# drtconway/zotmer

Hardware: AMD Instinct MI355X
Metric: Gk-mers/sec kmerize k=25 on synthetic 150bp FASTQ; achieved HBM GB/s fraction (higher is better)
Workload: dtype u64

## Files before the change

### zotmer_amd/csrc/stream_pass.hip

```cpp
#include "internal.hpp"
#include "encode_tile.hpp"

#include <stdlib.h>
#include <type_traits>

namespace zk {

constexpr int P0_BLOCK = 512, P0_NW = 8, P0_TILE = P0_BLOCK * P0_NW, P0_IMG_WORDS = 320;
constexpr int PW_BLOCK = 1024, PW_NW = 8, PW_TILE = PW_BLOCK * PW_NW, PW_IMG_WORDS = 640;
constexpr int SH_BLOCK = 512, SH_NW = 16, SH_TILE = SH_BLOCK * SH_NW;

struct P0Geom { u32 block, nw, img_words; };
__host__ __device__ constexpr P0Geom p0_geom(bool wide) { return wide ? P0Geom{PW_BLOCK, PW_NW, PW_IMG_WORDS} : P0Geom{P0_BLOCK, P0_NW, P0_IMG_WORDS}; }

struct StreamTiling {
    u32 rec;
    u32 rpt, cpr, wpr;
    u32 cpr_inv;
    u32 tile_bytes;
    u32 ranges;
    u64 range_bytes;
};

__host__ __device__ inline StreamTiling make_tiling(u64 n_bytes, u64 first_nl, int K, u32 ranges, P0Geom g) {
    StreamTiling t = {};
    const u32 tile = g.block * g.nw;
    t.ranges = ranges ? ranges : 1;
    t.tile_bytes = tile;
    if (first_nl < 0x7fffffffull) {
        const u64 rec = first_nl + 1;
        const long long W = (long long)first_nl - K + 1;
        if (rec >= 16 && W >= 1 && n_bytes % rec == 0) {
            const u32 cpr = (u32)((W + g.nw - 1) / g.nw);
            u32 rpt = cpr <= g.block ? (g.block / cpr) / 16 * 16 : 0;
            const u32 fit = (u32)((16ull * (g.img_words - 3)) / rec) / 16 * 16;
            if (rpt > fit) rpt = fit;
            if (rpt >= 16 && (u64)rpt * rec * 50 > (u64)tile * 51) {
                t.rec = (u32)rec; t.rpt = rpt; t.cpr = cpr; t.wpr = (u32)W;
                t.cpr_inv = (u32)(((1ull << 32) + cpr - 1) / cpr);
                t.tile_bytes = rpt * (u32)rec;
            }
        }
    }
    const u64 tiles = (n_bytes + t.tile_bytes - 1) / t.tile_bytes;
    const u64 tpr = (tiles + t.ranges - 1) / t.ranges;
    t.range_bytes = (tpr ? tpr : 1) * (u64)t.tile_bytes;
    return t;
}

__device__ __forceinline__ void encode_swar16(const uint4 q, u32& codes, u32& vmask) {
    const u32 w[4] = {q.x, q.y, q.z, q.w};
    u32 cc = 0, vv = 0;
#pragma unroll
    for (int i = 0; i < 4; i++) {
        const u32 t = (w[i] >> 1) & 0x03030303u;
        const u32 code = t ^ ((t >> 1) & 0x01010101u);
        const u32 g = (code | (code >> 6) | (code >> 12) | (code >> 18)) & 0xffu;
        cc |= g << (8 * i);
        const u32 x = w[i] | 0x20202020u;
        const u32 t1 = (x >> 2) & ~(x >> 1);
        const u32 b4 = x >> 4;
        const u32 inner = (b4 & t1) | (~b4 & x & ~t1);
        const u32 ok = ~(x >> 7) & (x >> 6) & ~(x >> 3) & inner & 0x01010101u;
// ... 20 lines not shown
    u32 s0, s1, s2;
    u32 r0, r1, r2;
    __device__ __forceinline__ void init(u64 a, u64 b, u32 s, int K) {
        shr128(a, b, 128u - 2u * s - 2u * (NW - 1) - 2u * (u32)K, s0, s1, s2);
        const u64 rhi = rev_pairs(~b), rlo = rev_pairs(~a);
        shr128(rhi, rlo, 2u * s, r0, r1, r2);
    }
    __device__ __forceinline__ u32 xhi(int i) const { return __builtin_amdgcn_alignbit(s2, s1, 2 * (NW - 1 - i)); }
    __device__ __forceinline__ u32 xlo(int i) const { return __builtin_amdgcn_alignbit(s1, s0, 2 * (NW - 1 - i)); }
    __device__ __forceinline__ u32 bhi(int i) const { return __builtin_amdgcn_alignbit(r2, r1, 2 * i); }
    __device__ __forceinline__ u32 blo(int i) const { return __builtin_amdgcn_alignbit(r1, r0, 2 * i); }
};

__device__ __forceinline__ u64 runs_of_k(u64 v, int K) {
    int have = 1;
    while (2 * have <= K) { v &= v << have; have *= 2; }
    v &= v << (K - have);
    return v;
}

__device__ __forceinline__ u32 spread16(u32 x) {
    x = (x | (x << 8)) & 0x00FF00FFu;
    x = (x | (x << 4)) & 0x0F0F0F0Fu;
    x = (x | (x << 2)) & 0x33333333u;
    x = (x | (x << 1)) & 0x55555555u;
    return x;
}

struct SHistArgs {
    const u8* stream;
    u64 n_bytes;
    int K, mode;
    PassPlan plan;
    u32 binbase[MAX_PASSES];
    u32 nbins;
    u64* ghist;
    u32 gstride;
    u32* rows;
    u64* acgt;
    u64* rec_info;
    u64* sample;
    u32* sample_n;
    u32 sample_cap;
    int sample_shift;
    u64 sample_value;
    u32 revbase;
    u32 ranges, split;
    u32* gcodes;
    u16* gvalid;
    int dbg_atomics;
    P0Geom geom;
};

template <bool HI, bool TWO, int CANON_T = -1>
__global__ __launch_bounds__(SH_BLOCK, 4) void stream_hist_kernel(SHistArgs h) {
    extern __shared__ u32 bins[];
    __shared__ TileImage<SH_TILE> img;
    __shared__ u32 pshift[MAX_PASSES], pmask[MAX_PASSES], pbase[MAX_PASSES];
    const int tid = threadIdx.x;
    for (u32 i = tid; i < h.nbins; i += SH_BLOCK) bins[i] = 0;
    if (tid < MAX_PASSES) {
        pshift[tid] = (u32)h.plan.shift[tid] - (HI ? 32u : 0u);
        pmask[tid] = (1u << h.plan.bits[tid]) - 1u;
        pbase[tid] = h.binbase[tid];
    }
    const u64 first_nl = h.rec_info[0];
    const StreamTiling tl = make_tiling(h.n_bytes, first_nl, h.K, h.ranges, h.geom);
    const u32 w = blockIdx.x / h.split, sp = blockIdx.x % h.split;
    const u64 B = (u64)w * tl.range_bytes;
    const u64 E = (B + tl.range_bytes < h.n_bytes) ? B + tl.range_bytes : h.n_bytes;
    const u32 ntile = B < E ? (u32)((E - B + SH_TILE - 1) / SH_TILE) : 0u;
    const int K = h.K;
    const int np = h.plan.passes;
    const u64 mask = ~0ull >> (64 - 2 * K);
    const u32 mlo = (u32)mask, mhi = (u32)(mask >> 32);
    const bool canon = CANON_T == 1 ? true : h.mode == ZK_KEYS_CANONICAL;
    const bool both = CANON_T != 1 && h.mode == ZK_KEYS_BOTH;
    const u32 sh0 = (u32)h.plan.shift[0] - (HI ? 32u : 0u), sh1 = (u32)h.plan.shift[1] - (HI ? 32u : 0u);
    const u32 dm0 = (1u << h.plan.bits[0]) - 1u, dm1 = (1u << h.plan.bits[1]) - 1u;
    const u32 base1 = h.binbase[1];
    const u32 nb0 = (u32)h.plan.bits[0], nb1 = (u32)h.plan.bits[1];
    const u32 ssh = (u32)h.sample_shift - (HI ? 32u : 0u);
    const typename std::conditional<HI, u32, u64>::type sval = (typename std::conditional<HI, u32, u64>::type)h.sample_value;
    u32 a0 = 0, a1 = 0, a2 = 0, a3 = 0, nl_count = 0, bad_count = 0;
    u32 rec = 0, m = 0, step_m = 0;
    if (first_nl < 0x7fffffffull) {
        rec = (u32)first_nl + 1u;
        m = (u32)((B + (u64)sp * SH_TILE + 16ull * tid) % rec);
        step_m = (u32)(((u64)h.split * SH_TILE) % rec);
    }
    uint4 q0 = make_uint4(0, 0, 0, 0), q1 = q0;
    auto issue = [&](u32 j) {
        const u64 P = B + (u64)j * SH_TILE;
        q0 = load_chunk16(h.stream, h.n_bytes, P + 16ull * tid);
        if (tid < 3) q1 = load_chunk16(h.stream, h.n_bytes, P + 16ull * (tid + SH_BLOCK));
    };
    if (sp < ntile) issue(sp);
    __syncthreads();
    for (u32 j = sp; j < ntile; j += h.split) {
        const u64 off = B + (u64)j * SH_TILE + 16ull * tid;
        const bool mine = off < E;
        {
            u32 cc, vv;
            encode_swar16(q0, cc, vv);
            if (rec) {
                if (mine) {
                    const int sep = (int)(rec - 1u) - (int)m;
                    const bool expect = sep >= 0 && sep < 16 && off + (u64)sep < h.n_bytes;
                    const u32 sepbit = expect ? (0x8000u >> (sep & 15)) : 0u;
                    if ((vv | sepbit) == 0xffffu) {
                        const u32 wsel = (sep & 12) == 0 ? q0.x : (sep & 12) == 4 ? q0.y : (sep & 12) == 8 ? q0.z : q0.w;
                        const bool isnl = ((wsel >> (8 * (sep & 3))) & 0xffu) == 0x0au;
                        nl_count += (expect && isnl) ? 1u : 0u;
                        bad_count += (expect && !isnl) ? 1u : 0u;
                    } else {
                        const u32 w4[4] = {q0.x, q0.y, q0.z, q0.w};
                        bool bad = false;
#pragma unroll
                        for (int q = 0; q < 4; q++) {
                            const u32 x = w4[q] ^ 0x0a0a0a0au;
                            const u32 t = ~(((x & 0x7f7f7f7fu) + 0x7f7f7f7fu) | x | 0x7f7f7f7fu);
                            nl_count += (u32)__popc(t);
                            const u32 want = (expect && (sep >> 2) == q) ? (0x80u << (8 * (sep & 3))) : 0u;
                            bad |= (t != want);
                        }
                        bad_count += bad ? 1u : 0u;
                    }
                }
                m += step_m;
                if (m >= rec) m -= rec;
            }
            img.codes[tid] = cc; img.valid[tid] = vv;
            if (mine && h.gcodes) { h.gcodes[off >> 4] = cc; h.gvalid[off >> 4] = (u16)vv; }
            if (tid < 3) {
                encode_swar16(q1, cc, vv);
                img.codes[tid + SH_BLOCK] = cc; img.valid[tid + SH_BLOCK] = vv;
            }
        }
        __syncthreads();
        if (j + h.split < ntile) issue(j + h.split);
        const u64 a = ((u64)img.codes[tid] << 32) | img.codes[tid + 1];
        const u64 b = ((u64)img.codes[tid + 2] << 32) | img.codes[tid + 3];
        u64 v = ((u64)img.valid[tid] << 48) | ((u64)img.valid[tid + 1] << 32) | ((u64)img.valid[tid + 2] << 16) | (u64)img.valid[tid + 3];
        v = runs_of_k(v, K);
        const u32 V16 = mine ? (u32)(v >> 48) : 0u;
        WindowWords<SH_NW> ww;
        ww.init(a, b, 0u, K);
        if (h.acgt) {
            const u32 Vs = spread16(V16);
            const u32 ff = (u32)(a >> 32);
            const u32 fl = (u32)((K > 1 ? ((a << (2 * K - 2)) | (b >> (66 - 2 * K))) : a) >> 32);
            const u32 lf = ff & Vs, hf = (ff >> 1) & Vs, ll = fl & Vs, hl = (fl >> 1) & Vs;
            a0 += (u32)__popc(Vs & ~hl & ~ll) + (u32)__popc(hf & lf);
            a1 += (u32)__popc(~hl & ll) + (u32)__popc(hf & ~lf);
            a2 += (u32)__popc(hl & ~ll) + (u32)__popc(~hf & lf);
            a3 += (u32)__popc(hl & ll) + (u32)__popc(Vs & ~hf & ~lf);
        }
        u32 hits = 0;
#pragma unroll
        for (int i = 0; i < SH_NW; i++) {
            const u32 inc = (V16 >> (15 - i)) & 1u;
            typename std::conditional<HI, u32, u64>::type kd;
            if constexpr (HI) {
                const u32 xh = ww.xhi(i) & mhi, bh = ww.bhi(i) & mhi;
                kd = canon ? (xh < bh ? xh : bh) : xh;
            } else {
                const u64 x = ((u64)(ww.xhi(i) & mhi) << 32) | (ww.xlo(i) & mlo), xb = ((u64)(ww.bhi(i) & mhi) << 32) | (ww.blo(i) & mlo);
                kd = canon ? (x < xb ? x : xb) : x;
            }
            if constexpr (TWO && HI) {
#ifdef ZK_PHASES
                if (h.dbg_atomics >= 1) atomicAdd(&bins[__builtin_amdgcn_ubfe(kd, sh0, nb0)], inc);
                if (h.dbg_atomics >= 2) atomicAdd(&bins[base1 + __builtin_amdgcn_ubfe(kd, sh1, nb1)], inc);
                if (h.dbg_atomics == 0) a0 += kd & inc;
#else
                atomicAdd(&bins[__builtin_amdgcn_ubfe(kd, sh0, nb0)], inc);
                atomicAdd(&bins[base1 + __builtin_amdgcn_ubfe(kd, sh1, nb1)], inc);
#endif
            } else if constexpr (TWO) {
                atomicAdd(&bins[(u32)(kd >> sh0) & dm0], inc);
                atomicAdd(&bins[base1 + ((u32)(kd >> sh1) & dm1)], inc);
            } else {
                for (int p = 0; p < np; p++) atomicAdd(&bins[pbase[p] + ((u32)(kd >> pshift[p]) & pmask[p])], inc);
                if (both) {
                    typename std::conditional<HI, u32, u64>::type kr;
                    if constexpr (HI) kr = ww.bhi(i) & mhi;
                    else kr = ((u64)(ww.bhi(i) & mhi) << 32) | (ww.blo(i) & mlo);
                    atomicAdd(&bins[h.revbase + ((u32)(kr >> pshift[0]) & pmask[0])], inc);
                    for (int p = 1; p < np; p++) atomicAdd(&bins[pbase[p] + ((u32)(kr >> pshift[p]) & pmask[p])], inc);
                }
            }
            if constexpr (HI) {
                if (h.sample) hits |= ((kd >> ssh) == sval ? 1u : 0u) << (15 - i);
            } else if (h.sample && inc && (kd >> ssh) == sval) {
                const u32 at = atomicAdd(h.sample_n, 1u);
                if (at < h.sample_cap) h.sample[at] = kd;
            }
        }
        hits &= V16;
        if (HI && hits) {
#pragma unroll
            for (int i = 0; i < SH_NW; i++) {
                if ((hits >> (15 - i)) & 1u) {
                    const u64 x = (((u64)ww.xhi(i) << 32) | ww.xlo(i)) & mask, xb = (((u64)ww.bhi(i) << 32) | ww.blo(i)) & mask;
                    const u64 kk = canon ? (x < xb ? x : xb) : x;
                    const u32 at = atomicAdd(h.sample_n, 1u);
                    if (at < h.sample_cap) h.sample[at] = kk;
                }
            }
        }
        __syncthreads();
    }
    __syncthreads();
    const u32 r0 = 1u << h.plan.bits[0];
    for (u32 i = tid; i < h.nbins; i += SH_BLOCK) {
        const u32 c = bins[i];
        if (!c) continue;
        if (i < r0) atomicAdd(&h.rows[(u64)w * r0 + i], c);
        if (both && i >= h.revbase) {
            atomicAdd(&h.rows[(u64)(h.ranges + w) * r0 + (i - h.revbase)], c);
            atomicAdd(&h.ghist[i - h.revbase], (u64)c);
            continue;
        }
        int p = 0;
        for (int q = 1; q < np; q++) if (i >= pbase[q]) p = q;
        atomicAdd(&h.ghist[(u64)p * h.gstride + (i - pbase[p])], (u64)c);
    }
    if (rec) {
        nl_count = wave_sum_u32(nl_count); bad_count = wave_sum_u32(bad_count);
        if ((tid & 63) == 0) {
            if (nl_count) atomicAdd(&h.rec_info[1], (u64)nl_count);
            if (bad_count) atomicAdd(&h.rec_info[2], (u64)bad_count);
        }
    }
    if (h.acgt) {
        a0 = wave_sum_u32(a0); a1 = wave_sum_u32(a1); a2 = wave_sum_u32(a2); a3 = wave_sum_u32(a3);
        if ((tid & 63) == 0) {
            if (a0) atomicAdd(&h.acgt[0], (u64)a0);
            if (a1) atomicAdd(&h.acgt[1], (u64)a1);
            if (a2) atomicAdd(&h.acgt[2], (u64)a2);
            if (a3) atomicAdd(&h.acgt[3], (u64)a3);
        }
    }
}

__global__ void rows_scan_kernel(const u32* __restrict__ rows, const u64* __restrict__ ghist0, u32 ranges, u32 radix, u64* __restrict__ offs) {
    const u32 d = blockIdx.x * blockDim.x + threadIdx.x;
    if (d >= radix) return;
    u64 run = ghist0[d];
    for (u32 w = 0; w < ranges; w++) {
        offs[(u64)w * radix + d] = run;
        run += rows[(u64)w * radix + d];
    }
}

struct P0Args {
    const u32* gcodes;
    const u16* gvalid;
    u64 n_bytes;
    int K;
// ... 181 lines not shown
            u32 e4[NF];
            u32 d8[NF][4];
            u64 b4[NF];
#pragma unroll
            for (int g = 0; g < NF; g++) {
                const u32 u = base + g * BLOCK + (u32)tid;
                e4[g] = sm.units[u < (u32)S::UNITS ? u : 0u];
            }
#pragma unroll
            for (int g = 0; g < NF; g++) asm volatile("" : "+v"(e4[g]));
#pragma unroll
            for (int g = 0; g < NF; g++) {
                const u32 sl = e4[g] & 0x3fffu;
                u32 hw[8];
#pragma unroll
                for (int q = 0; q < 8; q++) hw[q] = (u32)(sm.exch[sl + q] >> 32);
#pragma unroll
                for (int q = 0; q < 4; q++)
                    d8[g][q] = ((hw[2 * q] >> (a.dig_shift - 32)) & a.dig_mask) | (((hw[2 * q + 1] >> (a.dig_shift - 32)) & a.dig_mask) << 16);
                b4[g] = sm.gbase[(e4[g] >> 18) & (u32)(RADIX - 1)];
            }
#pragma unroll
            for (int g = 0; g < NF; g++) asm volatile("" : "+v"(d8[g][0]), "+v"(d8[g][1]), "+v"(d8[g][2]), "+v"(d8[g][3]), "+v"(b4[g]));
#pragma unroll
            for (int g = 0; g < NF; g++) {
                const u32 u = base + g * BLOCK + (u32)tid;
                const u32 len = ((e4[g] >> 14) & 15u) + 1u;
                u16* dst = a.dig_out + (b4[g] + (e4[g] & 0x3fffu));
                if (u < end && P0_MODE != 1) {
                    if (len == 8) { Dig8 v; v.a = d8[g][0]; v.b = d8[g][1]; v.c = d8[g][2]; v.d = d8[g][3]; *reinterpret_cast<Dig8*>(dst) = v; }
                    else {
#pragma unroll
                        for (int q = 0; q < 7; q++) if ((u32)q < len) dst[q] = (u16)(d8[g][q >> 1] >> (16 * (q & 1)));
                    }
                }
            }
        }
    };
    u32 held = 0, held_end = 0;
    for (u32 t = 0; t < ntile; t++) {
        const u64 T0 = B + (u64)t * tile_bytes;
        const bool last = t + 1 == ntile;
        if (P0_MODE == 2 && t > 1) {
            __syncthreads();
            sm.gbase[tid] += flen_dbg;
            __syncthreads();
        } else {
        u64 key[NW];
        u32 live;
        {
            const u32 j = p0 >> 4, s = p0 & 15u;
            const u64 sa = ((u64)sm.codes[j] << 32) | sm.codes[j + 1];
            const u64 sb = ((u64)sm.codes[j + 2] << 32) | sm.codes[j + 3];
            u64 v = ((u64)sm.valid[j] << 48) | ((u64)sm.valid[j + 1] << 32) | ((u64)sm.valid[j + 2] << 16) | (u64)sm.valid[j + 3];
            v = runs_of_k(v, K);
            live = (__brev((u32)((v << s) >> (64 - NW))) >> (32 - NW)) & wlim;
            if (T0 + p0 >= E) live = 0;
            WindowWords<NW> ww;
            ww.init(sa, sb, s, K);
#pragma unroll
            for (int i = 0; i < NW; i++) {
                const u64 x = ((u64)(ww.xhi(i) & mhi) << 32) | (FAST ? ww.xlo(i) : (ww.xlo(i) & mlo));
                if constexpr (CANON) {
                    const u64 xb = ((u64)(ww.bhi(i) & mhi) << 32) | (FAST ? ww.blo(i) : (ww.blo(i) & mlo));
                    key[i] = x < xb ? x : xb;
                } else {
                    const u64 xb = ((u64)(ww.bhi(i) & mhi) << 32) | (FAST ? ww.blo(i) : (ww.blo(i) & mlo));
                    key[i] = rev ? xb : x;
                }
            }
        }
        u64 ck[G - 1];
#pragma unroll
        for (int j = 0; j < G - 1; j++) ck[j] = sm.exch[ctail + j];
        u32 rk[NW];
#pragma unroll
        for (int i = 0; i < NW; i++) {
            rk[i] = atomicAdd(&sm.cnt[((live >> i) & 1u) ? digit(key[i]) : (u32)RADIX + (u32)lane], 1u);
        }
        if constexpr (!PLANES) { if (held < held_end) store_units(held, held_end, std::integral_constant<int, 2>()); }
        held = held_end = 0;
        P0_PHASE(0);
        __syncthreads();
        P0_PHASE(1);
        u32 O, tot, flen, head, nu;
        {
            const uint4 c0 = reinterpret_cast<const uint4*>(sm.cnt)[2 * lane], c1 = reinterpret_cast<const uint4*>(sm.cnt)[2 * lane + 1];
            const u32 s8 = c0.x + c0.y + c0.z + c0.w + c1.x + c1.y + c1.z + c1.w;
            const u32 inc8 = wave_incl_scan_dpp(s8);
            const u32 before = wave ? (u32)__builtin_amdgcn_readlane((int)inc8, 8 * wave - 1) : 0u;
            tot = sm.cnt[tid];
            const u32 inc = wave_incl_scan_dpp(tot);
            O = before + inc - tot;
            u64 end = F + tot;
            if (end > Fend) { bad = 1; sm.anybad = 1; end = Fend > F ? Fend : F; }
            u64 Eo = last ? end : (end & ~(u64)(G - 1));
            if (Eo < F) Eo = F;
            flen = (u32)(Eo - F);
            head = (u32)(F & (G - 1)) ? G - (u32)(F & (G - 1)) : 0u;
            if (head > flen) head = flen;
            nu = (head ? 1u : 0u) + (flen - head + G - 1) / G;
            sm.nu[tid] = (u16)nu;
        }
        __syncthreads();
        {
            const uint4 c0 = reinterpret_cast<const uint4*>(sm.nu)[lane];
            const u32 s2 = c0.x + c0.y + c0.z + c0.w;
            const u32 s8 = (s2 & 0xffffu) + (s2 >> 16);
            const u32 inc8 = wave_incl_scan_dpp(s8);
// ... 139 lines not shown
    (void)tlast;
    struct __attribute__((packed, aligned(8))) Key2 { u64 a, b; };
    auto store_units = [&](u32 end) {
        constexpr int NF = 2;
        constexpr u32 LPU = G / 2, GROUPS = BLOCK / LPU;
        const u32 j = 2u * ((u32)tid & (LPU - 1)), g0 = (u32)tid / LPU;
        for (u32 base = 0; base < end; base += NF * GROUPS) {
            u32 e4[NF];
            u64 k4[NF], l4[NF], b4[NF];
#pragma unroll
            for (int g = 0; g < NF; g++) {
                const u32 u = base + g * GROUPS + g0;
                e4[g] = sm.units[u < end ? u : 0u];
            }
#pragma unroll
            for (int g = 0; g < NF; g++) asm volatile("" : "+v"(e4[g]));
#pragma unroll
            for (int g = 0; g < NF; g++) {
                const u32 d = (e4[g] >> 18) & (u32)(RADIX - 1), kc = e4[g] >> 27;
                const u32 cs = (u32)S::CB + (u32)S::CARRY * d, ps = (e4[g] & 0x3fffu) - 16u;
                k4[g] = sm.exch[j < kc ? cs + j : ps + j];
                l4[g] = sm.exch[j + 1 < kc ? cs + j + 1 : ps + j + 1];
                b4[g] = sm.gbase[d];
            }
#pragma unroll
            for (int g = 0; g < NF; g++) asm volatile("" : "+v"(k4[g]), "+v"(l4[g]), "+v"(b4[g]));
#pragma unroll
            for (int g = 0; g < NF; g++) {
                const u32 u = base + g * GROUPS + g0;
                const u32 len1 = (e4[g] >> 14) & 15u;
                u64* dst = a.kout + (b4[g] + (e4[g] & 0x3fffu) + j);
                const bool fits = P0_MODE != 2 || b4[g] + (e4[g] & 0x3fffu) + G <= a.n;
                if (u < end && P0_MODE != 1 && fits) {
                    if (j < len1) { Key2 v; v.a = k4[g]; v.b = l4[g]; *reinterpret_cast<Key2*>(dst) = v; }
                    else if (j == len1) *dst = k4[g];
                }
            }
        }
    };
    for (u32 t = 0; t < ntile; t++) {
        const u64 T0 = B + (u64)t * tile_bytes;
        const bool last = t + 1 == ntile;
        if (P0_MODE == 2 && t > 1) {
            __syncthreads();
            if (owner) sm.gbase[tid] += flen_dbg;
            __syncthreads();
        } else {
        u64 key[NW];
        u32 live;
        {
            const u32 j = p0 >> 4, s = p0 & 15u;
            const u64 sa = ((u64)sm.codes[j] << 32) | sm.codes[j + 1];
            const u64 sb = ((u64)sm.codes[j + 2] << 32) | sm.codes[j + 3];
            u64 v = ((u64)sm.valid[j] << 48) | ((u64)sm.valid[j + 1] << 32) | ((u64)sm.valid[j + 2] << 16) | (u64)sm.valid[j + 3];
            v = runs_of_k(v, K);
            live = (__brev((u32)((v << s) >> (64 - NW))) >> (32 - NW)) & wlim;
            if (T0 + p0 >= E) live = 0;
            WindowWords<NW> ww;
            ww.init(sa, sb, s, K);
#pragma unroll
            for (int i = 0; i < NW; i++) {
                const u64 x = ((u64)(ww.xhi(i) & mhi) << 32) | (FAST ? ww.xlo(i) : (ww.xlo(i) & mlo));
                const u64 xb = ((u64)(ww.bhi(i) & mhi) << 32) | (FAST ? ww.blo(i) : (ww.blo(i) & mlo));
                if constexpr (CANON) key[i] = x < xb ? x : xb;
                else key[i] = rev ? xb : x;
            }
        }
        u32 rk[NW];
#pragma unroll
        for (int i = 0; i < NW; i++) rk[i] = atomicAdd(&sm.cnt[((live >> i) & 1u) ? digit(key[i]) : (u32)RADIX + (u32)lane], 1u);
        P0_PHASE(0);
        __syncthreads();
        P0_PHASE(1);
        u32 O = 0, tot = 0, flen = 0, head = 0, nu = 0, c = 0;
        if (owner) {
            const uint4 c0 = reinterpret_cast<const uint4*>(sm.cnt)[2 * lane], c1 = reinterpret_cast<const uint4*>(sm.cnt)[2 * lane + 1];
            const u32 s8 = c0.x + c0.y + c0.z + c0.w + c1.x + c1.y + c1.z + c1.w;
            const u32 inc8 = wave_incl_scan_dpp(s8);
            const u32 before = wave ? (u32)__builtin_amdgcn_readlane((int)inc8, 8 * wave - 1) : 0u;
            c = sm.cnt[tid];
            const u32 inc = wave_incl_scan_dpp(c);
            O = before + inc - c;
            tot = r + c;
            u64 end = F + tot;
            if (end > Fend) { bad = 1; sm.anybad = 1; end = Fend > F ? Fend : F; }
            u64 Eo = last ? end : (end & ~(u64)(G - 1));
            if (Eo < F) Eo = F;
            flen = (u32)(Eo - F);
            head = (u32)(F & (G - 1)) ? G - (u32)(F & (G - 1)) : 0u;
            if (head > flen) head = flen;
            nu = (head ? 1u : 0u) + (flen - head + G - 1) / G;
            sm.off[tid] = (u16)O;
            sm.nu[tid] = (u16)nu;
        } else {
            const u32 q = (u32)tid - (u32)RADIX, j = 2u * (q & 7u);
#pragma unroll
            for (int h = 0; h < 2; h++) {
                u32 m4[4], d4[4];
                u64 v4[4], x4[4];
#pragma unroll
                for (int g = 0; g < 4; g++) { d4[g] = (u32)(4 * h + g) * (RADIX / 8) + (q >> 3); m4[g] = sm.mv[d4[g]]; }
#pragma unroll
                for (int g = 0; g < 4; g++) asm volatile("" : "+v"(m4[g]));
#pragma unroll
                for (int g = 0; g < 4; g++) {
                    const u32 n = m4[g] >> 18, src = m4[g] & 0x3fffu;
                    v4[g] = sm.exch[j < n ? src + j : (u32)S::DEAD + (u32)lane];
                    x4[g] = sm.exch[j + 1 < n ? src + j + 1 : (u32)S::DEAD + (u32)lane];
                }
// ... 33 lines not shown
                const u32 kc = i < r ? (r - i < len ? r - i : len) : 0u;
                if (U < (u32)S::UNITS) sm.units[U] = unit_pack(ps + i, len, (u32)tid) | (kc << 27);
                U++; i += len; left -= len;
            }
            const u32 keep = tot - flen;
            u32 src = O, dsto = r, n = c;
            if (flen && flen >= r) { src = O + flen - r; dsto = 0; n = keep; }
            if (dsto > (u32)S::CARRY) dsto = S::CARRY;
            if (n > (u32)S::CARRY - dsto) n = (u32)S::CARRY - dsto;
            sm.mv[tid] = src | (dsto << 14) | (n << 18);
            r = keep < (u32)S::CARRY ? keep : (u32)S::CARRY;
            sm.cnt[tid] = 0;
            F += flen;
        }
        {
            u32 at[NW];
#pragma unroll
            for (int i = 0; i < NW; i++) at[i] = sm.off[digit(key[i])];
#pragma unroll
            for (int i = 0; i < NW; i++) sm.exch[((live >> i) & 1u) ? at[i] + rk[i] : (u32)S::DEAD + (u32)lane] = key[i];
        }
        if (!last) {
            if ((u32)tid < nch) { sm.codes[tid] = qc; sm.valid[tid] = qv; }
            if (t + 2 < ntile) fetch(T0 + 2ull * tile_bytes);
        }
        P0_PHASE(4);
        __syncthreads();
        P0_PHASE(5);
        }
        {
            const u32 nunits = (sm.anybad || sm.nunits > (u32)S::UNITS) ? 0u : sm.nunits;
            store_units(nunits);
        }
        P0_PHASE(6);
    }
    if (a.dbg && tid == 0) {
        for (int k = 0; k < 8; k++) a.dbg[(u64)w * 16 + k] = (u64)ph[k];
        a.dbg[(u64)w * 16 + 8] = ntile;
    }
    if (P0_MODE) return;
    if (bad || (mine && (F != Fend || r != 0))) atomicOr(a.err, ZK_DERR_MISMATCH);
}

static bool p0_wide(const zk_ctx* c) { return (c->stream_pass & 0xff) == 1 && !c->tag_pass; }

int stream_ranges(zk_ctx* c, bool wide) { return c->stream_ranges > 0 ? c->stream_ranges : (wide ? 1 : 2) * (c->num_cus > 0 ? c->num_cus : 1); }

int stream_hist(zk_ctx* c, const u8* stream, uint64_t n_bytes, int K, int mode, const PassPlan& plan, u64* ghist, u32 gstride,
                u64* d_acgt, u64* d_n, u64* rec_info, u64* sample, u32 sample_cap, int sample_shift, u64 sample_value, u32* sample_n,
                void* image_room, uint64_t image_room_bytes, StreamRows* out) {
    SHistArgs h = {};
    h.stream = stream; h.n_bytes = n_bytes; h.K = K; h.mode = mode; h.plan = plan;
    u32 nb = 0;
    bool hi = 2 * K > 32;
    for (int p = 0; p < plan.passes; p++) { h.binbase[p] = nb; nb += 1u << plan.bits[p]; if (plan.shift[p] < 32) hi = false; }
    if (sample && sample_shift < 32) hi = false;
    const bool both = mode == ZK_KEYS_BOTH;
    const u32 strands = both ? 2u : 1u;
    h.revbase = nb;
    if (both) nb += 1u << plan.bits[0];
    h.nbins = nb;
    h.ghist = ghist; h.gstride = gstride;
    h.acgt = d_acgt; h.rec_info = rec_info;
    h.sample = sample; h.sample_n = sample_n; h.sample_cap = sample_cap; h.sample_shift = sample_shift; h.sample_value = sample_value;
    const bool wide = p0_wide(c);
    h.geom = p0_geom(wide);
    h.ranges = (u32)stream_ranges(c, wide);
    h.split = wide ? 8 : 4;
    h.dbg_atomics = 2;
#ifdef ZK_PHASES
    if (const char* e = getenv("ZK_HIST_ATOMICS")) h.dbg_atomics = atoi(e);
#endif
    const u32 r0 = 1u << plan.bits[0];
    const uint64_t nchunks = (n_bytes + 15) / 16;
    u32* rows; u64* offs;
    ZK_TRY(arena_alloc(c, sizeof(u32) * (uint64_t)strands * h.ranges * r0, (void**)&rows));
    ZK_TRY(arena_alloc(c, sizeof(u64) * (uint64_t)strands * h.ranges * r0, (void**)&offs));
    const uint64_t codes_bytes = (sizeof(u32) * nchunks + 255) & ~255ull, image_bytes = codes_bytes + ((sizeof(u16) * nchunks + 255) & ~255ull);
    char* img = nullptr;
    if (image_room && image_room_bytes >= image_bytes + 256) img = (char*)(((uintptr_t)image_room + image_room_bytes - image_bytes) & ~(uintptr_t)255);
    else ZK_TRY(arena_alloc(c, image_bytes, (void**)&img));
    h.gcodes = (u32*)img; h.gvalid = (u16*)(img + codes_bytes);
    h.rows = rows;
    ZK_HIP(c, hipMemsetAsync(rows, 0, sizeof(u32) * (uint64_t)strands * h.ranges * r0, c->stream));
    ZK_HIP(c, hipMemsetAsync(ghist, 0, sizeof(u64) * MAX_PASSES * gstride, c->stream));
    if (d_acgt) ZK_HIP(c, hipMemsetAsync(d_acgt, 0, sizeof(u64) * 4, c->stream));
    const u32 grid = h.ranges * h.split;
    prof_begin(c, ZK_PROF_HIST_STREAM, n_bytes);
    const bool two = plan.passes == 2 && !both;
    if (hi && two && mode == ZK_KEYS_CANONICAL) hipLaunchKernelGGL((stream_hist_kernel<true, true, 1>), dim3(grid), dim3(SH_BLOCK), nb * sizeof(u32), c->stream, h);
    else if (hi && two) hipLaunchKernelGGL((stream_hist_kernel<true, true>), dim3(grid), dim3(SH_BLOCK), nb * sizeof(u32), c->stream, h);
    else if (hi) hipLaunchKernelGGL((stream_hist_kernel<true, false>), dim3(grid), dim3(SH_BLOCK), nb * sizeof(u32), c->stream, h);
    else if (two) hipLaunchKernelGGL((stream_hist_kernel<false, true>), dim3(grid), dim3(SH_BLOCK), nb * sizeof(u32), c->stream, h);
    else hipLaunchKernelGGL((stream_hist_kernel<false, false>), dim3(grid), dim3(SH_BLOCK), nb * sizeof(u32), c->stream, h);
    prof_end(c);
    ZK_HIP(c, hipGetLastError());
    out->rows = rows; out->offs = offs; out->ranges = h.ranges; out->strands = strands; out->radix = r0; out->gcodes = h.gcodes; out->gvalid = h.gvalid;
    out->wide = wide;
    return ZK_OK;
}

int stream_pass0(zk_ctx* c, uint64_t n_bytes, int K, int mode, int shift, int bits, const u64* ghist0, const StreamRows& rows,
                 uint64_t first_nl, bool uniform, u64* kout, uint64_t n, int variant, const StreamPlanes* planes) {
    if (bits < 1 || bits > 9 || (1u << bits) != rows.radix) return fail(c, ZK_EINTERNAL, "stream_pass0: %d digit bits, rows of %u", bits, rows.radix);
    if ((mode == ZK_KEYS_BOTH) != (rows.strands == 2)) return fail(c, ZK_EINTERNAL, "stream_pass0: rows of %u strands for mode %d", rows.strands, mode);
    const u32 grid = rows.ranges * rows.strands;
    hipLaunchKernelGGL(rows_scan_kernel, dim3((rows.radix + 255) / 256), dim3(256), 0, c->stream, rows.rows, ghist0, grid, rows.radix, rows.offs);
    P0Args a = {};
    a.gcodes = rows.gcodes; a.gvalid = rows.gvalid; a.n_bytes = n_bytes; a.K = K;
    a.tl = make_tiling(n_bytes, first_nl, K, rows.ranges, p0_geom(rows.wide));
    a.ranges = rows.ranges;
    a.by_record = (uniform && a.tl.rec) ? 1 : 0;
    a.shift = shift; a.bits = bits; a.offs = rows.offs; a.rows = rows.rows; a.kout = kout; a.n = n; a.err = c->d_err; a.dbg = c->dbg; a.dbg_mode = variant >> 8; a.split_stores = (variant & 0xff) == 3;
    const bool canon = mode == ZK_KEYS_CANONICAL, fast = 2 * K > 32 && shift >= 32;
    if (planes) {
        if (!canon || !fast || rows.wide) return fail(c, ZK_EINTERNAL, "stream_pass0: planes need the canonical fast plan and the 512-thread kernel");
        a.dig_out = planes->dig; a.dig_shift = planes->shift; a.dig_mask = (1u << planes->bits) - 1u;
        prof_begin(c, ZK_PROF_PASS_STREAM, n_bytes + 6 * n);
        hipLaunchKernelGGL((stream_pass0_kernel<9, 8, true, true, true>), dim3(rows.ranges), dim3(P0_BLOCK), 0, c->stream, a);
        prof_end(c);
        ZK_HIP(c, hipGetLastError());
// ... 19 lines not shown
```

Baseline: 168.9.

## Restructure stream histogram kernel: 32 windows per thread, prefix-based keys, precomputed validity

Shrinks the histogram block to 128 threads that each handle two 16-byte chunks (32 k-mer windows), with a larger split factor so more blocks cover each range. Keys in the high path now come from the top 32 bits of the k-mer (the shift follows 2K-32) through cheap alignbit prefix extraction, and the full 64-bit key is rebuilt only when a sample candidate is possible. The global validity image now holds the run-of-k mask, so the later partition kernels skip recomputing runs_of_k. This aims to cut per-window ALU work and LDS traffic, at the cost of more registers per thread and changed occupancy and tiling behaviour.

```diff
diff --git a/zotmer_amd/csrc/stream_pass.hip b/zotmer_amd/csrc/stream_pass.hip
--- a/zotmer_amd/csrc/stream_pass.hip
+++ b/zotmer_amd/csrc/stream_pass.hip
@@ -8,7 +8,7 @@
 
 constexpr int P0_BLOCK = 512, P0_NW = 8, P0_TILE = P0_BLOCK * P0_NW, P0_IMG_WORDS = 320;
 constexpr int PW_BLOCK = 1024, PW_NW = 8, PW_TILE = PW_BLOCK * PW_NW, PW_IMG_WORDS = 640;
-constexpr int SH_BLOCK = 512, SH_NW = 16, SH_TILE = SH_BLOCK * SH_NW;
+constexpr int SH_BLOCK = 128, SH_NW = 32, SH_TILE = SH_BLOCK * SH_NW;
 
 struct P0Geom { u32 block, nw, img_words; };
 __host__ __device__ constexpr P0Geom p0_geom(bool wide) { return wide ? P0Geom{PW_BLOCK, PW_NW, PW_IMG_WORDS} : P0Geom{P0_BLOCK, P0_NW, P0_IMG_WORDS}; }
@@ -135,15 +135,63 @@
     P0Geom geom;
 };
 
+struct HistWords {
+    u32 s0, s1, s2, s3;
+    u32 r0, r1, r2, r3;
+    __device__ __forceinline__ void init(u64 a, u64 b, u64 rlo, u64 rhi, int K) {
+        const u32 t = 66u - 2u * (u32)K;
+        const u64 lo = t == 64u ? a : ((b >> (t & 63u)) | (a << ((64u - t) & 63u)));
+        const u64 hi = t == 64u ? 0ull : (a >> (t & 63u));
+        s0 = (u32)lo; s1 = (u32)(lo >> 32); s2 = (u32)hi; s3 = (u32)(hi >> 32);
+        r0 = (u32)rlo; r1 = (u32)(rlo >> 32); r2 = (u32)rhi; r3 = (u32)(rhi >> 32);
+    }
+    __device__ __forceinline__ u32 xlo(int i) const { return i >= 16 ? __builtin_amdgcn_alignbit(s1, s0, 2 * (31 - i)) : __builtin_amdgcn_alignbit(s2, s1, 2 * (15 - i)); }
+    __device__ __forceinline__ u32 xhi(int i) const { return i >= 16 ? __builtin_amdgcn_alignbit(s2, s1, 2 * (31 - i)) : __builtin_amdgcn_alignbit(s3, s2, 2 * (15 - i)); }
+    __device__ __forceinline__ u32 blo(int i) const { return i < 16 ? __builtin_amdgcn_alignbit(r1, r0, 2 * i) : __builtin_amdgcn_alignbit(r2, r1, 2 * (i - 16)); }
+    __device__ __forceinline__ u32 bhi(int i) const { return i < 16 ? __builtin_amdgcn_alignbit(r2, r1, 2 * i) : __builtin_amdgcn_alignbit(r3, r2, 2 * (i - 16)); }
+};
+
+struct HistPrefixes {
+    u32 c0, c1, c2;
+    u32 r0, r1, r2;
+    __device__ __forceinline__ void init(u64 a, u64 b, u64 rlo, u64 rhi, u32 lead) {
+        c0 = (u32)(a >> 32); c1 = (u32)a; c2 = (u32)(b >> 32);
+        r0 = (u32)(rlo >> lead);
+        r1 = (u32)((((u64)(u32)rhi << 32) | (rlo >> 32)) >> lead);
+        r2 = (u32)(rhi >> lead);
+    }
+    __device__ __forceinline__ u32 fwd(int i) const {
+        return i == 0 ? c0 : i < 16 ? __builtin_amdgcn_alignbit(c0, c1, 32 - 2 * i) : i == 16 ? c1 : __builtin_amdgcn_alignbit(c1, c2, 64 - 2 * i);
+    }
+    __device__ __forceinline__ u32 rev(int i) const { return i < 16 ? __builtin_amdgcn_alignbit(r1, r0, 2 * i) : __builtin_amdgcn_alignbit(r2, r1, 2 * (i - 16)); }
+};
+
+__device__ __forceinline__ void hist_full_key(u64 a, u64 b, u64 rlo, u64 rhi, u32 i, int K, u64& x, u64& xb) {
+    const u64 mask = ~0ull >> (64 - 2 * K);
+    u32 w0, w1, w2;
+    shr128(a, b, 128u - 2u * i - 2u * (u32)K, w0, w1, w2);
+    x = (((u64)w1 << 32) | w0) & mask;
+    shr128(rhi, rlo, 2u * i, w0, w1, w2);
+    xb = (((u64)w1 << 32) | w0) & mask;
+}
+
+struct SHistImage {
+    static constexpr int NCH = SH_TILE / 16 + 4;
+    alignas(8) u32 codes[NCH];
+    alignas(8) u32 valid[NCH];
+};
+
 template <bool HI, bool TWO, int CANON_T = -1>
 __global__ __launch_bounds__(SH_BLOCK, 4) void stream_hist_kernel(SHistArgs h) {
     extern __shared__ u32 bins[];
-    __shared__ TileImage<SH_TILE> img;
+    __shared__ SHistImage img;
     __shared__ u32 pshift[MAX_PASSES], pmask[MAX_PASSES], pbase[MAX_PASSES];
     const int tid = threadIdx.x;
+    const int K = h.K;
+    const u32 lead = HI ? (u32)(2 * K - 32) : 0u;
     for (u32 i = tid; i < h.nbins; i += SH_BLOCK) bins[i] = 0;
     if (tid < MAX_PASSES) {
-        pshift[tid] = (u32)h.plan.shift[tid] - (HI ? 32u : 0u);
+        pshift[tid] = (u32)h.plan.shift[tid] - lead;
         pmask[tid] = (1u << h.plan.bits[tid]) - 1u;
         pbase[tid] = h.binbase[tid];
     }
@@ -153,142 +201,165 @@
     const u64 B = (u64)w * tl.range_bytes;
     const u64 E = (B + tl.range_bytes < h.n_bytes) ? B + tl.range_bytes : h.n_bytes;
     const u32 ntile = B < E ? (u32)((E - B + SH_TILE - 1) / SH_TILE) : 0u;
-    const int K = h.K;
     const int np = h.plan.passes;
     const u64 mask = ~0ull >> (64 - 2 * K);
     const u32 mlo = (u32)mask, mhi = (u32)(mask >> 32);
     const bool canon = CANON_T == 1 ? true : h.mode == ZK_KEYS_CANONICAL;
     const bool both = CANON_T != 1 && h.mode == ZK_KEYS_BOTH;
-    const u32 sh0 = (u32)h.plan.shift[0] - (HI ? 32u : 0u), sh1 = (u32)h.plan.shift[1] - (HI ? 32u : 0u);
+    const u32 sh0 = (u32)h.plan.shift[0] - lead, sh1 = (u32)h.plan.shift[1] - lead;
     const u32 dm0 = (1u << h.plan.bits[0]) - 1u, dm1 = (1u << h.plan.bits[1]) - 1u;
     const u32 base1 = h.binbase[1];
     const u32 nb0 = (u32)h.plan.bits[0], nb1 = (u32)h.plan.bits[1];
-    const u32 ssh = (u32)h.sample_shift - (HI ? 32u : 0u);
-    const typename std::conditional<HI, u32, u64>::type sval = (typename std::conditional<HI, u32, u64>::type)h.sample_value;
+    const u32 ssh = h.sample ? (u32)h.sample_shift - lead : 0u;
+    const u32 svall = HI ? (u32)h.sample_value << (ssh & 31u) : 0u, slim = HI ? 1u << (ssh & 31u) : 0u;
+    const u64 sval = h.sample_value;
     u32 a0 = 0, a1 = 0, a2 = 0, a3 = 0, nl_count = 0, bad_count = 0;
-    u32 rec = 0, m = 0, step_m = 0;
+    u32 rec = 0, m = 0, step_m = 0, m16 = 0;
     if (first_nl < 0x7fffffffull) {
         rec = (u32)first_nl + 1u;
-        m = (u32)((B + (u64)sp * SH_TILE + 16ull * tid) % rec);
+        m = (u32)((B + (u64)sp * SH_TILE + 32ull * tid) % rec);
         step_m = (u32)(((u64)h.split * SH_TILE) % rec);
-    }
-    uint4 q0 = make_uint4(0, 0, 0, 0), q1 = q0;
+        m16 = 16u % rec;
+    }
+    auto check_chunk = [&](const uint4 q, u32 vv, u64 off, u32 mm) {
+        const int sep = (int)(rec - 1u) - (int)mm;
+        const bool expect = sep >= 0 && sep < 16 && off + (u64)sep < h.n_bytes;
+        const u32 sepbit = expect ? (0x8000u >> (sep & 15)) : 0u;
+        if ((vv | sepbit) == 0xffffu) {
+            const u32 wsel = (sep & 12) == 0 ? q.x : (sep & 12) == 4 ? q.y : (sep & 12) == 8 ? q.z : q.w;
+            const bool isnl = ((wsel >> (8 * (sep & 3))) & 0xffu) == 0x0au;
+            nl_count += (expect && isnl) ? 1u : 0u;
+            bad_count += (expect && !isnl) ? 1u : 0u;
+        } else {
+            const u32 w4[4] = {q.x, q.y, q.z, q.w};
+            bool bad = false;
+#pragma unroll
+            for (int k = 0; k < 4; k++) {
+                const u32 x = w4[k] ^ 0x0a0a0a0au;
+                const u32 t = ~(((x & 0x7f7f7f7fu) + 0x7f7f7f7fu) | x | 0x7f7f7f7fu);
+                nl_count += (u32)__popc(t);
+                const u32 want = (expect && (sep >> 2) == k) ? (0x80u << (8 * (sep & 3))) : 0u;
+                bad |= (t != want);
+            }
+            bad_count += bad ? 1u : 0u;
+        }
+    };
+    uint4 q0 = make_uint4(0, 0, 0, 0), q1 = q0, qh = q0;
     auto issue = [&](u32 j) {
         const u64 P = B + (u64)j * SH_TILE;
-        q0 = load_chunk16(h.stream, h.n_bytes, P + 16ull * tid);
-        if (tid < 3) q1 = load_chunk16(h.stream, h.n_bytes, P + 16ull * (tid + SH_BLOCK));
+        q0 = load_chunk16(h.stream, h.n_bytes, P + 32ull * tid);
+        q1 = load_chunk16(h.stream, h.n_bytes, P + 32ull * tid + 16ull);
+        if (tid < 3) qh = load_chunk16(h.stream, h.n_bytes, P + (u64)SH_TILE + 16ull * tid);
     };
     if (sp < ntile) issue(sp);
     __syncthreads();
     for (u32 j = sp; j < ntile; j += h.split) {
-        const u64 off = B + (u64)j * SH_TILE + 16ull * tid;
-        const bool mine = off < E;
-        {
+        const u64 off0 = B + (u64)j * SH_TILE + 32ull * tid, off1 = off0 + 16ull;
+        const bool mine0 = off0 < E, mine1 = off1 < E;
+        u32 cc0, vv0, cc1, vv1;
+        encode_swar16(q0, cc0, vv0);
+        encode_swar16(q1, cc1, vv1);
+        if (rec) {
+            if (mine0) check_chunk(q0, vv0, off0, m);
+            if (mine1) { const u32 mm = m + m16; check_chunk(q1, vv1, off1, mm >= rec ? mm - rec : mm); }
+            m += step_m;
+            if (m >= rec) m -= rec;
+        }
+        *reinterpret_cast<uint2*>(&img.codes[2 * tid]) = make_uint2(cc0, cc1);
+        *reinterpret_cast<uint2*>(&img.valid[2 * tid]) = make_uint2(vv0, vv1);
+        if (h.gcodes) {
+            if (mine0) h.gcodes[off0 >> 4] = cc0;
+            if (mine1) h.gcodes[off1 >> 4] = cc1;
+        }
+        if (tid < 3) {
             u32 cc, vv;
-            encode_swar16(q0, cc, vv);
-            if (rec) {
-                if (mine) {
-                    const int sep = (int)(rec - 1u) - (int)m;
-                    const bool expect = sep >= 0 && sep < 16 && off + (u64)sep < h.n_bytes;
-                    const u32 sepbit = expect ? (0x8000u >> (sep & 15)) : 0u;
-                    if ((vv | sepbit) == 0xffffu) {
-                        const u32 wsel = (sep & 12) == 0 ? q0.x : (sep & 12) == 4 ? q0.y : (sep & 12) == 8 ? q0.z : q0.w;
-                        const bool isnl = ((wsel >> (8 * (sep & 3))) & 0xffu) == 0x0au;
-                        nl_count += (expect && isnl) ? 1u : 0u;
-                        bad_count += (expect && !isnl) ? 1u : 0u;
-                    } else {
-                        const u32 w4[4] = {q0.x, q0.y, q0.z, q0.w};
-                        bool bad = false;
-#pragma unroll
-                        for (int q = 0; q < 4; q++) {
-                            const u32 x = w4[q] ^ 0x0a0a0a0au;
-                            const u32 t = ~(((x & 0x7f7f7f7fu) + 0x7f7f7f7fu) | x | 0x7f7f7f7fu);
-                            nl_count += (u32)__popc(t);
-                            const u32 want = (expect && (sep >> 2) == q) ? (0x80u << (8 * (sep & 3))) : 0u;
-                            bad |= (t != want);
-                        }
-                        bad_count += bad ? 1u : 0u;
+            encode_swar16(qh, cc, vv);
+            img.codes[SH_TILE / 16 + tid] = cc; img.valid[SH_TILE / 16 + tid] = vv;
+        }
+        __syncthreads();
+        if (j + h.split < ntile) issue(j + h.split);
+        const uint2 nc = *reinterpret_cast<const uint2*>(&img.codes[2 * tid + 2]), nv = *reinterpret_cast<const uint2*>(&img.valid[2 * tid + 2]);
+        const u64 a = ((u64)cc0 << 32) | cc1, b = ((u64)nc.x << 32) | nc.y;
+        u64 v = ((u64)vv0 << 48) | ((u64)vv1 << 32) | ((u64)nv.x << 16) | (u64)nv.y;
+        v = runs_of_k(v, K);
+        const u32 W32 = (u32)(v >> 32);
+        if (h.gvalid) {
+            if (mine0) h.gvalid[off0 >> 4] = (u16)(W32 >> 16);
+            if (mine1) h.gvalid[off1 >> 4] = (u16)W32;
+        }
+        const u32 V32 = W32 & ((mine0 ? 0xffff0000u : 0u) | (mine1 ? 0x0000ffffu : 0u));
+        const u64 rlo = rev_pairs(~a), rhi = rev_pairs(~b);
+        if (h.acgt) {
+            const u64 Vs = ((u64)spread16(V32 >> 16) << 32) | spread16(V32 & 0xffffu);
+            const u64 ff = a;
+            const u64 fl = K > 1 ? ((a << (2 * K - 2)) | (b >> (66 - 2 * K))) : a;
+            const u64 lf = ff & Vs, hf = (ff >> 1) & Vs, ll = fl & Vs, hl = (fl >> 1) & Vs;
+            a0 += (u32)__popcll(Vs & ~hl & ~ll) + (u32)__popcll(hf & lf);
+            a1 += (u32)__popcll(~hl & ll) + (u32)__popcll(hf & ~lf);
+            a2 += (u32)__popcll(hl & ~ll) + (u32)__popcll(~hf & lf);
+            a3 += (u32)__popcll(hl & ll) + (u32)__popcll(Vs & ~hf & ~lf);
+        }
+        if constexpr (HI) {
+            HistPrefixes pw;
+            pw.init(a, b, rlo, rhi, lead);
+            u32 smin = ~0u;
+#pragma unroll
+            for (int i = 0; i < SH_NW; i++) {
+                const u32 inc = (V32 >> (31 - i)) & 1u;
+                const u32 pf = pw.fwd(i), pb = pw.rev(i);
+                const u32 kd = canon ? (pf < pb ? pf : pb) : pf;
+                if constexpr (TWO) {
+#ifdef ZK_PHASES
+                    if (h.dbg_atomics >= 1) atomicAdd(&bins[__builtin_amdgcn_ubfe(kd, sh0, nb0)], inc);
+                    if (h.dbg_atomics >= 2) atomicAdd(&bins[base1 + __builtin_amdgcn_ubfe(kd, sh1, nb1)], inc);
+                    if (h.dbg_atomics == 0) a0 += kd & inc;
+#else
+                    atomicAdd(&bins[__builtin_amdgcn_ubfe(kd, sh0, nb0)], inc);
+                    atomicAdd(&bins[base1 + __builtin_amdgcn_ubfe(kd, sh1, nb1)], inc);
+#endif
+                } else {
+                    for (int p = 0; p < np; p++) atomicAdd(&bins[pbase[p] + ((kd >> pshift[p]) & pmask[p])], inc);
+                    if (both) {
+                        atomicAdd(&bins[h.revbase + ((pb >> pshift[0]) & pmask[0])], inc);
+                        for (int p = 1; p < np; p++) atomicAdd(&bins[pbase[p] + ((pb >> pshift[p]) & pmask[p])], inc);
                     }
                 }
-                m += step_m;
-                if (m >= rec) m -= rec;
-            }
-            img.codes[tid] = cc; img.valid[tid] = vv;
-            if (mine && h.gcodes) { h.gcodes[off >> 4] = cc; h.gvalid[off >> 4] = (u16)vv; }
-            if (tid < 3) {
-                encode_swar16(q1, cc, vv);
-                img.codes[tid + SH_BLOCK] = cc; img.valid[tid + SH_BLOCK] = vv;
-            }
-        }
-        __syncthreads();
-        if (j + h.split < ntile) issue(j + h.split);
-        const u64 a = ((u64)img.codes[tid] << 32) | img.codes[tid + 1];
-        const u64 b = ((u64)img.codes[tid + 2] << 32) | img.codes[tid + 3];
-        u64 v = ((u64)img.valid[tid] << 48) | ((u64)img.valid[tid + 1] << 32) | ((u64)img.valid[tid + 2] << 16) | (u64)img.valid[tid + 3];
-        v = runs_of_k(v, K);
-        const u32 V16 = mine ? (u32)(v >> 48) : 0u;
-        WindowWords<SH_NW> ww;
-        ww.init(a, b, 0u, K);
-        if (h.acgt) {
-            const u32 Vs = spread16(V16);
-            const u32 ff = (u32)(a >> 32);
-            const u32 fl = (u32)((K > 1 ? ((a << (2 * K - 2)) | (b >> (66 - 2 * K))) : a) >> 32);
-            const u32 lf = ff & Vs, hf = (ff >> 1) & Vs, ll = fl & Vs, hl = (fl >> 1) & Vs;
-            a0 += (u32)__popc(Vs & ~hl & ~ll) + (u32)__popc(hf & lf);
-            a1 += (u32)__popc(~hl & ll) + (u32)__popc(hf & ~lf);
-            a2 += (u32)__popc(hl & ~ll) + (u32)__popc(~hf & lf);
-            a3 += (u32)__popc(hl & ll) + (u32)__popc(Vs & ~hf & ~lf);
-        }
-        u32 hits = 0;
-#pragma unroll
-        for (int i = 0; i < SH_NW; i++) {
-            const u32 inc = (V16 >> (15 - i)) & 1u;
-            typename std::conditional<HI, u32, u64>::type kd;
-            if constexpr (HI) {
-                const u32 xh = ww.xhi(i) & mhi, bh = ww.bhi(i) & mhi;
-                kd = canon ? (xh < bh ? xh : bh) : xh;
-            } else {
+                const u32 sx = kd ^ svall;
+                smin = sx < smin ? sx : smin;
+            }
+            if (h.sample && smin < slim) {
+#pragma unroll 1
+                for (u32 i = 0; i < (u32)SH_NW; i++) {
+                    u64 x, xb;
+                    hist_full_key(a, b, rlo, rhi, i, K, x, xb);
+                    const u64 kk = canon ? (x < xb ? x : xb) : x;
+                    if (((V32 >> (31u - i)) & 1u) && (kk >> h.sample_shift) == sval) {
+                        const u32 at = atomicAdd(h.sample_n, 1u);
+                        if (at < h.sample_cap) h.sample[at] = kk;
+                    }
+                }
+            }
+        } else {
+            HistWords ww;
+            ww.init(a, b, rlo, rhi, K);
+#pragma unroll
+            for (int i = 0; i < SH_NW; i++) {
+                const u32 inc = (V32 >> (31 - i)) & 1u;
                 const u64 x = ((u64)(ww.xhi(i) & mhi) << 32) | (ww.xlo(i) & mlo), xb = ((u64)(ww.bhi(i) & mhi) << 32) | (ww.blo(i) & mlo);
-                kd = canon ? (x < xb ? x : xb) : x;
-            }
-            if constexpr (TWO && HI) {
-#ifdef ZK_PHASES
-                if (h.dbg_atomics >= 1) atomicAdd(&bins[__builtin_amdgcn_ubfe(kd, sh0, nb0)], inc);
-                if (h.dbg_atomics >= 2) atomicAdd(&bins[base1 + __builtin_amdgcn_ubfe(kd, sh1, nb1)], inc);
-                if (h.dbg_atomics == 0) a0 += kd & inc;
-#else
-                atomicAdd(&bins[__builtin_amdgcn_ubfe(kd, sh0, nb0)], inc);
-                atomicAdd(&bins[base1 + __builtin_amdgcn_ubfe(kd, sh1, nb1)], inc);
-#endif
-            } else if constexpr (TWO) {
-                atomicAdd(&bins[(u32)(kd >> sh0) & dm0], inc);
-                atomicAdd(&bins[base1 + ((u32)(kd >> sh1) & dm1)], inc);
-            } else {
-                for (int p = 0; p < np; p++) atomicAdd(&bins[pbase[p] + ((u32)(kd >> pshift[p]) & pmask[p])], inc);
-                if (both) {
-                    typename std::conditional<HI, u32, u64>::type kr;
-                    if constexpr (HI) kr = ww.bhi(i) & mhi;
-                    else kr = ((u64)(ww.bhi(i) & mhi) << 32) | (ww.blo(i) & mlo);
-                    atomicAdd(&bins[h.revbase + ((u32)(kr >> pshift[0]) & pmask[0])], inc);
-                    for (int p = 1; p < np; p++) atomicAdd(&bins[pbase[p] + ((u32)(kr >> pshift[p]) & pmask[p])], inc);
+                const u64 kd = canon ? (x < xb ? x : xb) : x;
+                if constexpr (TWO) {
+                    atomicAdd(&bins[(u32)(kd >> sh0) & dm0], inc);
+                    atomicAdd(&bins[base1 + ((u32)(kd >> sh1) & dm1)], inc);
+                } else {
+                    for (int p = 0; p < np; p++) atomicAdd(&bins[pbase[p] + ((u32)(kd >> pshift[p]) & pmask[p])], inc);
+                    if (both) {
+                        atomicAdd(&bins[h.revbase + ((u32)(xb >> pshift[0]) & pmask[0])], inc);
+                        for (int p = 1; p < np; p++) atomicAdd(&bins[pbase[p] + ((u32)(xb >> pshift[p]) & pmask[p])], inc);
+                    }
                 }
-            }
-            if constexpr (HI) {
-                if (h.sample) hits |= ((kd >> ssh) == sval ? 1u : 0u) << (15 - i);
-            } else if (h.sample && inc && (kd >> ssh) == sval) {
-                const u32 at = atomicAdd(h.sample_n, 1u);
-                if (at < h.sample_cap) h.sample[at] = kd;
-            }
-        }
-        hits &= V16;
-        if (HI && hits) {
-#pragma unroll
-            for (int i = 0; i < SH_NW; i++) {
-                if ((hits >> (15 - i)) & 1u) {
-                    const u64 x = (((u64)ww.xhi(i) << 32) | ww.xlo(i)) & mask, xb = (((u64)ww.bhi(i) << 32) | ww.blo(i)) & mask;
-                    const u64 kk = canon ? (x < xb ? x : xb) : x;
+                if (h.sample && inc && (kd >> ssh) == sval) {
                     const u32 at = atomicAdd(h.sample_n, 1u);
-                    if (at < h.sample_cap) h.sample[at] = kk;
+                    if (at < h.sample_cap) h.sample[at] = kd;
                 }
             }
         }
@@ -576,9 +647,8 @@
             const u32 j = p0 >> 4, s = p0 & 15u;
             const u64 sa = ((u64)sm.codes[j] << 32) | sm.codes[j + 1];
             const u64 sb = ((u64)sm.codes[j + 2] << 32) | sm.codes[j + 3];
-            u64 v = ((u64)sm.valid[j] << 48) | ((u64)sm.valid[j + 1] << 32) | ((u64)sm.valid[j + 2] << 16) | (u64)sm.valid[j + 3];
-            v = runs_of_k(v, K);
-            live = (__brev((u32)((v << s) >> (64 - NW))) >> (32 - NW)) & wlim;
+            const u32 v = (sm.valid[j] << 16) | sm.valid[j + 1];
+            live = (__brev((v << s) >> (32 - NW)) >> (32 - NW)) & wlim;
             if (T0 + p0 >= E) live = 0;
             WindowWords<NW> ww;
             ww.init(sa, sb, s, K);
@@ -824,9 +894,8 @@
             const u32 j = p0 >> 4, s = p0 & 15u;
             const u64 sa = ((u64)sm.codes[j] << 32) | sm.codes[j + 1];
             const u64 sb = ((u64)sm.codes[j + 2] << 32) | sm.codes[j + 3];
-            u64 v = ((u64)sm.valid[j] << 48) | ((u64)sm.valid[j + 1] << 32) | ((u64)sm.valid[j + 2] << 16) | (u64)sm.valid[j + 3];
-            v = runs_of_k(v, K);
-            live = (__brev((u32)((v << s) >> (64 - NW))) >> (32 - NW)) & wlim;
+            const u32 v = (sm.valid[j] << 16) | sm.valid[j + 1];
+            live = (__brev((v << s) >> (32 - NW)) >> (32 - NW)) & wlim;
             if (T0 + p0 >= E) live = 0;
             WindowWords<NW> ww;
             ww.init(sa, sb, s, K);
@@ -966,9 +1035,9 @@
     SHistArgs h = {};
     h.stream = stream; h.n_bytes = n_bytes; h.K = K; h.mode = mode; h.plan = plan;
     u32 nb = 0;
-    bool hi = 2 * K > 32;
-    for (int p = 0; p < plan.passes; p++) { h.binbase[p] = nb; nb += 1u << plan.bits[p]; if (plan.shift[p] < 32) hi = false; }
-    if (sample && sample_shift < 32) hi = false;
+    bool hi = 2 * K >= 32;
+    for (int p = 0; p < plan.passes; p++) { h.binbase[p] = nb; nb += 1u << plan.bits[p]; if (plan.shift[p] < 2 * K - 32) hi = false; }
+    if (sample && (sample_shift < 2 * K - 32 || sample_shift >= 2 * K)) hi = false;
     const bool both = mode == ZK_KEYS_BOTH;
     const u32 strands = both ? 2u : 1u;
     h.revbase = nb;
@@ -980,7 +1049,7 @@
     const bool wide = p0_wide(c);
     h.geom = p0_geom(wide);
     h.ranges = (u32)stream_ranges(c, wide);
-    h.split = wide ? 8 : 4;
+    h.split = wide ? 64 : 32;
     h.dbg_atomics = 2;
 #ifdef ZK_PHASES
     if (const char* e = getenv("ZK_HIST_ATOMICS")) h.dbg_atomics = atoi(e);
```

New measurement: 171.3, median of 6. About the same (+1.4%).
